# maxvonbuelow/harry

Hardware: AMD Instinct MI355X
Metric: Mtriangles/s encode+decode (higher is better)
Workload: dtype u8/u16 residual bytes, u32 range-coder registers (compat profile: u64)

## Files before the change

harry_amd/csrc/device/chunked.cpp:

```cpp
#include <chrono>
#include <condition_variable>
#include <cstdio>
#include <cstdlib>
#include <cstring>
#include <deque>
#include <memory>
#include <mutex>
#include <thread>

#include "codec_math.hpp"
#include "context.hpp"
#include "kernels.hpp"

namespace hry {

using namespace dev;
static const char kMarkPrefix[] = "[hry enc]";

static constexpr int kDefaultChunk = 8192;
static constexpr uint32_t kMaxChunk = 1u << 20;


static uint32_t stream_words(uint32_t n, uint32_t t0)
{
// ... 539 lines not shown
		std::vector<RestartCounters> scounters;
		dir.restarts = select_restart_points(w.marks, w.named, dir.counters, &w.snapshots, &scounters);
		if (!w.snapshots.empty()) write_snapshot_section(w.snapshot_faces, w.snapshots, scounters, dir.snapshot_section);
		write_restart_section(dir, restart_sec);
	};
	const bool dir_beside = w.marks.size() >= 4096 && host_threads() > 1;
	SideThreads dir_helper;
	if (dir_beside) dir_helper.spawn(select_restarts);

	const uint32_t vc = (uint32_t)w.order_v.size(), fc = (uint32_t)w.order_f.size();
	if (piped && (vc != pipe->vc || fc != pipe->fc)) throw Error(HRY_E_INTERNAL, "encode pipeline: sizes changed under the walk");
	if (chunk_syms <= 0) {
		uint64_t total = (uint64_t)w.n_conn + (uint64_t)vc * ldv.nplanes + (uint64_t)fc * ldf.nplanes;
		if (m.general) for (const AttrList &L : m.lists) total += (uint64_t)L.count * L.coded_bytes();
		while (CH < (1u << 15) && total / CH > 8192) CH <<= 1;
	}

	auto t_h2d = Clock::now();
	size_t op_plane_n[8];
	for (int k = 0; k < 8; ++k) op_plane_n[k] = w.n_op_class[k];
	size_t ngrp = 0, conn_plane_bytes = 0, nopb = w.op_sc.size();
	for (int g = 0; g < G_COUNT; ++g) { ngrp += w.grp_val[g].size(); conn_plane_bytes += w.grp_val[g].size() * kGroupBytes[g]; }
	cx.d_order_v.ensure(std::max<size_t>((size_t)vc * 4, 16));
	cx.d_order_f.ensure(std::max<size_t>((size_t)fc * 4, 16));
	cx.d_rank.ensure(std::max<size_t>((size_t)dev_nv * 4, 16));
	cx.d_grp_val.ensure(std::max<size_t>(ngrp * 4, 16));
	cx.d_connplanes.ensure(std::max<size_t>(conn_plane_bytes + 2 * nopb + 64, 16));
	cx.d_vplanes.ensure(std::max<size_t>((size_t)vc * ldv.nplanes, 16));
	cx.d_fplanes.ensure(std::max<size_t>((size_t)fc * ldf.nplanes, 16));
	const bool nt_piped = piped && pipe->nt != nullptr;
	if (vc && !piped) HIP_OK(hipMemcpyAsync(cx.d_order_v.p, w.order_v.data(), (size_t)vc * 4, hipMemcpyHostToDevice, cx.stream));
	if (fc && (ldf.nplanes || m.general) && !piped) HIP_OK(hipMemcpyAsync(cx.d_order_f.p, w.order_f.data(), (size_t)fc * 4, hipMemcpyHostToDevice, cx.stream));
	if (!piped) upload_repaired_twins(cx, in_place ? *in_place->whole : m, w, in_place != nullptr);
	if (in_place) cx.inplace_twin_patches.insert(cx.inplace_twin_patches.end(), w.twin_patches.begin(), w.twin_patches.end());
	size_t goff[G_COUNT + 1] = { 0 };
	for (int g = 0; g < G_COUNT; ++g) {
		size_t n = w.grp_val[g].size();
		goff[g + 1] = goff[g] + n;
		if (n && !(g == G_NUMTRI && nt_piped)) HIP_OK(hipMemcpyAsync(cx.d_grp_val.as<uint32_t>() + goff[g], w.grp_val[g].data(), n * 4, hipMemcpyHostToDevice, cx.stream));
	}
	uint8_t *d_opplanes = cx.d_connplanes.as<uint8_t>() + conn_plane_bytes;
	uint8_t *d_opraw = d_opplanes + nopb;
	if (nopb) HIP_OK(hipMemcpyAsync(d_opraw, w.op_sc.data(), nopb, hipMemcpyHostToDevice, cx.stream));

	const std::vector<GenPlane> layout = container_planes(m);
	std::vector<PlaneRef> planes;
	auto add_plane = [&](const uint8_t *at, uint32_t n) { planes.push_back(PlaneRef{ at, n, layout.at(planes.size()).init }); };
	{
		size_t poff = 0;
		for (int g = 0; g < G_COUNT; ++g) {
			uint32_t n = (uint32_t)w.grp_val[g].size();
			const uint8_t *at = g == G_NUMTRI && nt_piped ? cx.d_nt_planes.as<uint8_t>() : cx.d_connplanes.as<uint8_t>() + poff;
			for (int b = 0; b < kGroupBytes[g]; ++b) add_plane(at + (size_t)b * n, n);
			poff += (size_t)n * kGroupBytes[g];
		}
		size_t o = 0;
		for (int k = 0; k < kOpClasses; ++k) { add_plane(d_opplanes + o, (uint32_t)op_plane_n[k]); o += op_plane_n[k]; }
		for (int p = 0; p < ldv.nplanes; ++p) add_plane(cx.d_vplanes.as<uint8_t>() + (size_t)p * vc, vc);
		for (int p = 0; p < ldf.nplanes; ++p) add_plane(cx.d_fplanes.as<uint8_t>() + (size_t)p * fc, fc);
	}
	if (m.general) general_planes_encode(cx, m, w, planes);
	if (planes.size() != layout.size()) throw Error(HRY_E_INTERNAL, "chunked encode: the planes do not match the container's layout");
	std::vector<uint32_t> kind_tabs;
	build_init_tables(m, kind_tabs);
	const uint32_t CHC = std::min(CH, std::max(CH / 8, 512u));
	dir.CH = CH; dir.CHC = CHC;
	const uint32_t npl = (uint32_t)planes.size();
	std::vector<HistSlice> slices;
	for (uint32_t pi = 0; pi < npl; ++pi)
		for (uint32_t f = 0; f < planes[pi].n; f += 16384) slices.push_back(HistSlice{ planes[pi].dptr + f, std::min(16384u, planes[pi].n - f), pi });
	cx.d_small.ensure(std::max<size_t>(slices.size() * sizeof(HistSlice) + (size_t)npl * 1024 + 64, 64));
	uint32_t *d_hist = cx.d_small.as<uint32_t>();
	HistSlice *d_slices = (HistSlice*)(cx.d_small.as<uint8_t>() + (size_t)npl * 1024);
	if (!slices.empty()) HIP_OK(hipMemcpyAsync(d_slices, slices.data(), slices.size() * sizeof(HistSlice), hipMemcpyHostToDevice, cx.stream));
	HIP_OK(hipMemsetAsync(d_hist, 0, (size_t)npl * 1024, cx.stream));
	HIP_OK(hipStreamSynchronize(cx.stream));
	cx.timing.h2d_ms = ms_since(t_h2d);
	HRY_MARK(t_all, "walk's outputs on the device");

	ConnView cv = cx.conn_view();
	HIP_OK(hipEventRecord(cx.ev[1], cx.stream));
	if (!m.general && !piped) {
		HIP_OK(hipMemsetAsync(cx.d_rank.p, 0xff, (size_t)dev_nv * 4, cx.stream));
		launch_rank(cx.stream, cx.d_order_v.as<uint32_t>(), vc, cv.org, cx.d_rank.as<uint32_t>());
		launch_predict_vtx(cx.stream, cv, cx.d_order_v.as<uint32_t>(), vc, cx.d_rank.as<uint32_t>(), cx.d_rec[1].as<uint8_t>(), ldv, cx.d_vplanes.as<uint8_t>());
		launch_face_planes(cx.stream, cv, cx.d_order_f.as<uint32_t>(), fc, cx.d_rec[0].as<uint8_t>(), ldf, cx.d_fplanes.as<uint8_t>());
	}
	{
		size_t poff = 0;
		for (int g = 0; g < G_COUNT; ++g) {
			uint32_t n = (uint32_t)w.grp_val[g].size();
			if (!(g == G_NUMTRI && nt_piped)) launch_split_bytes(cx.stream, cx.d_grp_val.as<uint32_t>() + goff[g], n, kGroupBytes[g], cx.d_connplanes.as<uint8_t>() + poff);
			poff += (size_t)n * kGroupBytes[g];
		}
	}
	{
		uint32_t base[8], o = 0;
		for (int k = 0; k < 8; ++k) { base[k] = o; o += (uint32_t)op_plane_n[k]; }
		cx.d_op.ensure(((nopb + kSplitUnit - 1) / kSplitUnit + 1) * 8 * 4 + 64);
		launch_split_classes(cx.stream, d_opraw, (uint32_t)nopb, base, cx.d_op.as<uint32_t>(), d_opplanes);
	}
	launch_plane_hist(cx.stream, d_slices, (uint32_t)slices.size(), d_hist);
	HIP_OK(hipEventRecord(cx.ev[2], cx.stream));
	std::vector<uint32_t> hist((size_t)npl * 256);
	if (npl) HIP_OK(hipMemcpyAsync(hist.data(), d_hist, hist.size() * 4, hipMemcpyDeviceToHost, cx.stream));
	HIP_OK(hipStreamSynchronize(cx.stream));
	HRY_MARK(t_all, "planes and their histograms");

	dir.tables.assign((size_t)npl * 256, 0);
	dir.has_prior.assign(npl, 0);
	dir.nsym.resize(npl);
	std::vector<uint32_t> totals(npl, 0);
	for (uint32_t pi = 0; pi < npl; ++pi) {
		uint32_t *tab = dir.tables.data() + (size_t)pi * 256;
		const bool use = plane_prior_from_hist(hist.data() + (size_t)pi * 256, planes[pi].n, tab);
		if (!use) memcpy(tab, kind_tabs.data() + (size_t)planes[pi].init * 256, 1024);
		for (int i = 0; i < 256; ++i) totals[pi] += tab[i];
		dir.has_prior[pi] = use ? 1 : 0;
		dir.nsym[pi] = planes[pi].n;
	}
	std::vector<StreamJob> jobs;
	uint64_t words = 0;
	uint64_t nsym_total = 0;
	uint32_t max_t0 = 256;
	for (uint32_t pi = 0; pi < npl; ++pi) {
		const PlaneRef &pl = planes[pi];
		nsym_total += pl.n;
		max_t0 = std::max(max_t0, totals[pi]);
		for_plane_streams(pi, pl.n, CH, CHC, [&](uint64_t f, uint32_t n) {
			if (words >= (1ull << 32) - (1u << 24)) throw Error(HRY_E_UNSUPPORTED, "chunked stream accumulator exceeds 2^32 words");
			jobs.push_back(StreamJob{ pl.dptr + f, n, pi, totals[pi], (uint32_t)words });
			words += stream_words(n, totals[pi]);
		});
	}
	const uint32_t ns = (uint32_t)jobs.size();
	const uint32_t nw = (uint32_t)words + 2;
	HRY_MARK(t_all, "  priors and stream jobs (host)");
	cx.d_init.ensure(std::max<size_t>(dir.tables.size() * 4, 16));
	if (!dir.tables.empty()) HIP_OK(hipMemcpyAsync(cx.d_init.p, dir.tables.data(), dir.tables.size() * 4, hipMemcpyHostToDevice, cx.stream));
	cx.d_cjobs.ensure(std::max<size_t>((size_t)ns * sizeof(StreamJob), 16));
	if (ns) HIP_OK(hipMemcpyAsync(cx.d_cjobs.p, jobs.data(), (size_t)ns * sizeof(StreamJob), hipMemcpyHostToDevice, cx.stream));
	cx.ensure_magic(max_t0 + CH + 16);
	cx.d_acc.ensure((size_t)nw * 8);
	cx.d_summary.ensure(((size_t)nw / 1024 + 8) * 4);
	cx.d_bytes.ensure((size_t)nw * 4);
	cx.d_csizes.ensure(std::max<size_t>((size_t)ns * 8, 16));
	cx.d_coffs.ensure(((size_t)ns + 1) * 8);
	HIP_OK(hipMemsetAsync(cx.d_acc.p, 0, (size_t)nw * 8, cx.stream));
	uint32_t *d_bits = cx.d_csizes.as<uint32_t>(), *d_nbytes = d_bits + ns;
	bool split_kernels;
	{
		uint32_t longest = 0;
		for (uint32_t i = 0; i < ns; ++i) longest = std::max(longest, jobs[i].n);
		const double one = std::max(longest * 0.09e-3, (double)nsym_total * 0.04e-6), two = longest * 0.207e-3 + (double)nsym_total * 0.0057e-6;
		const uint64_t min_streams = env_uint("HRY_ENCODE_SPLIT_MIN_STREAMS", ~0ull);
		split_kernels = min_streams != ~0ull ? min_streams != 0 && ns >= min_streams : ns >= 64 && two < 0.9 * one;
	}
	for (uint32_t i = 0; i < ns && split_kernels; ++i) split_kernels = (uint64_t)jobs[i].t0 + jobs[i].n <= 65535u;
	std::vector<uint64_t> tab;
	if (split_kernels) {
		tab.resize((size_t)ns + ((size_t)ns + 1) / 2);
		uint32_t *order = (uint32_t*)(tab.data() + ns);
		uint64_t off = 0;
		for (uint32_t i = 0; i < ns; ++i) { tab[i] = off; off += jobs[i].n; order[i] = i; }
		std::stable_sort(order, order + ns, [&](uint32_t a, uint32_t b) { return jobs[a].n > jobs[b].n; });
		cx.d_rec_sym.ensure(std::max<size_t>((size_t)off * 8, 16));
		cx.d_split.ensure(tab.size() * 8);
		HIP_OK(hipMemcpyAsync(cx.d_split.p, tab.data(), tab.size() * 8, hipMemcpyHostToDevice, cx.stream));
		HIP_OK(hipEventRecord(cx.ev[3], cx.stream));
		launch_chunk_encode_split(cx.stream, cx.d_cjobs.as<StreamJob>(), ns, cx.d_init.as<uint32_t>(), cx.d_magic.as<MagicEnt>(), cx.d_acc.as<uint64_t>(), d_bits,
		                          cx.d_split.as<uint64_t>(), cx.d_rec_sym.p, (const uint32_t*)(cx.d_split.as<uint64_t>() + ns));
		HIP_OK(hipEventRecord(cx.ev[4], cx.stream));
	} else {
	HIP_OK(hipEventRecord(cx.ev[3], cx.stream));
	launch_chunk_encode(cx.stream, cx.d_cjobs.as<StreamJob>(), ns, cx.d_init.as<uint32_t>(), cx.d_magic.as<MagicEnt>(), cx.d_acc.as<uint64_t>(), d_bits);
	HIP_OK(hipEventRecord(cx.ev[4], cx.stream));
	}
	launch_carry(cx.stream, cx.d_acc.as<uint64_t>(), nw, cx.d_v.as<uint64_t>(), cx.d_summary.as<uint32_t>(), cx.d_bytes.as<uint8_t>(), cx.d_cjobs.as<StreamJob>(), d_bits, ns);
	launch_stream_pack(cx.stream, cx.d_cjobs.as<StreamJob>(), ns, d_bits, nullptr, d_nbytes, cx.d_coffs.as<uint64_t>(), nullptr, false);
	cx.h_small.ensure(64);
	volatile uint64_t *total_bytes_p = cx.h_small.as<uint64_t>();
	*total_bytes_p = 0;
	HIP_OK(hipMemcpyAsync((void*)total_bytes_p, cx.d_coffs.as<uint64_t>() + ns, 8, hipMemcpyDeviceToHost, cx.stream));
	HRY_MARK(t_all, "  stream kernels launched");
	if (dir_beside) dir_helper.rethrow(); else select_restarts();
	HRY_MARK(t_all, "  restart points selected");
	HIP_OK(hipStreamSynchronize(cx.stream));
	const uint64_t total_bytes = *total_bytes_p;
	HRY_MARK(t_all, "streams coded");
	cx.d_cout.ensure(std::max<size_t>(total_bytes, 16));
	launch_stream_pack(cx.stream, cx.d_cjobs.as<StreamJob>(), ns, d_bits, cx.d_bytes.as<uint8_t>(), d_nbytes, cx.d_coffs.as<uint64_t>(), cx.d_cout.as<uint8_t>(), true);
	HIP_OK(hipEventRecord(cx.ev[5], cx.stream));

	write_container(cx, dir, restart_sec, ns, d_nbytes, total_bytes, out);
	HRY_MARK(t_all, "container on the host");
	if (sharded) { const uint64_t seg_len = out.size() - seg_begin; memcpy(out.data() + seg_len_at, &seg_len, 8); }

	if (cx.keep_stages) {
		cx.stage_put_host("order_v", w.order_v.data(), (size_t)vc * 4);
		cx.stage_put_host("order_f", w.order_f.data(), (size_t)fc * 4);
		cx.stage_put("vplanes", cx.d_vplanes.p, (size_t)vc * ldv.nplanes);
		cx.stage_put("fplanes", cx.d_fplanes.p, (size_t)fc * ldf.nplanes);
		cx.stage_put("d_twin", cx.d_twin.p, (size_t)(in_place ? in_place->whole->ne() : m.ne()) * 4);
	}
	cx.timing.k_predict_ms = cx.elapsed(1, 2);
	cx.timing.k_entropy_ms = cx.elapsed(3, 4);
	cx.timing.device_ms = cx.elapsed(1, 5);
	cx.timing.n_symbols = nsym_total;
	cx.timing.payload_bytes = total_bytes;
	cx.timing.total_ms = ms_since(t_all);
}

Mesh *decode_chunked(Context &cx, const uint8_t *p, size_t n, size_t hdr, std::unique_ptr<Mesh> m);
Mesh *decode_compat(Context &cx, const uint8_t *p, size_t n, size_t hdr, std::unique_ptr<Mesh> m);

Mesh *decode_any(Context &cx, const uint8_t *p, size_t n, int shard_index, int shard_count, bool allow_partial)
{
	HIP_OK(hipSetDevice(cx.device));
	std::unique_ptr<Mesh> m(new Mesh());
	int minor = 0;
	const bool sharded = n >= 6 && p[4] == 0 && p[5] == 3;
	size_t hdr = read_hry_header(p, n, *m, minor, !sharded);
	if (minor == 3) { Context *one = &cx; return decode_sharded(&one, 1, p, n, hdr, std::move(m), shard_index, shard_count, allow_partial || shard_count > 1, nullptr); }
	if (shard_count > 1) throw Error(HRY_E_ARG, "only a sharded container (.hry v0.3) decodes segment by segment");
	if (minor == 2) return decode_chunked(cx, p, n, hdr, std::move(m));
	if (m->general) return decode_general(cx, p, n, hdr, std::move(m));
	return decode_compat(cx, p, n, hdr, std::move(m));
}

}
```

harry_amd/csrc/device/chunked.hip:

```cpp
#include <hip/hip_runtime.h>

#include <mutex>
#include <stdexcept>
#include <type_traits>

#include "codec_math.hpp"
#include "dev_types.hpp"
#include "kernels.hpp"

namespace hry {
namespace dev {

__device__ __forceinline__ uint32_t wscan_excl(uint32_t v, uint32_t &total)
{
	uint32_t inc = v;
#pragma unroll
	for (int d = 1; d < 64; d <<= 1) {
		uint32_t o = __shfl_up(inc, d, 64);
		if ((int)(threadIdx.x & 63) >= d) inc += o;
	}
	total = __shfl(inc, 63, 64);
	return inc - v;
}

constexpr int kWin = 72;

__global__ __launch_bounds__(64) void k_chunk_encode(const StreamJob *jobs, const uint32_t *inits, const MagicEnt *magic,
                                                     unsigned long long *acc, uint32_t *stream_bits)
{
	const StreamJob jb = jobs[blockIdx.x];
	const int lane = threadIdx.x;
	__shared__ uint32_t cnt[257], cum[257], bh[256];
	__shared__ unsigned long long win[kWin];
	{
		const uint32_t *st = inits + (size_t)jb.init * 256 + 4 * lane;
		uint32_t a = st[0], b = st[1], c = st[2], d = st[3], tot;
		uint32_t ex = wscan_excl(a + b + c + d, tot);
		cnt[4 * lane] = a; cnt[4 * lane + 1] = b; cnt[4 * lane + 2] = c; cnt[4 * lane + 3] = d;
		cum[4 * lane] = ex; cum[4 * lane + 1] = ex + a; cum[4 * lane + 2] = ex + a + b; cum[4 * lane + 3] = ex + a + b + c;
		if (lane == 0) { cnt[256] = 0; cum[256] = 0; }
	}
	__syncthreads();
	uint32_t R = 1u << 31;
	uint32_t S = 0;
	const uint64_t earlier = lane == 0 ? 0ull : (~0ull >> (64 - lane));
	for (uint32_t base = 0; base < jb.n; base += 64) {
		const uint32_t j = base + lane;
		const bool valid = j < jb.n;
		const uint32_t nb = min(64u, jb.n - base);
		const uint32_t s = valid ? jb.sym[j] : 0x100u;
		uint64_t eq = ~0ull, lt = 0;
#pragma unroll
		for (int b = 8; b >= 0; --b) {
			const bool mine = (s >> b) & 1u;
			const uint64_t m = __ballot(mine);
			lt |= mine ? (eq & ~m) : 0ull;
			eq &= mine ? m : ~m;
		}
		const uint32_t l = cum[s] + (uint32_t)__popcll(lt & earlier), c = cnt[s] + (uint32_t)__popcll(eq & earlier);
		const uint32_t t = jb.t0 + j;
		const bool sub = l + c == t;
		MagicEnt me = valid ? magic[t] : MagicEnt{ 0, 0, 0 };
		const uint32_t mx = valid ? (sub ? l : c) : 0u;
		const uint32_t mm = ((me.shift >> kMagicSh32Shift) & 31u) | (sub || !valid ? 0x80u : 0u);
		uint32_t my_r = 0, my_s = 0;
		const uint32_t s_first = S;
		auto step = [&](uint32_t i) {
			const uint32_t M = (uint32_t)__builtin_amdgcn_readlane((int)me.m32, (int)i);
			const uint32_t x = (uint32_t)__builtin_amdgcn_readlane((int)mx, (int)i);
			const uint32_t meta = (uint32_t)__builtin_amdgcn_readlane((int)mm, (int)i);
			const uint32_t r = __umulhi(R, M) >> (meta & 31u);
			const uint32_t prod = r * x;
			const uint32_t Rn = (meta & 0x80u) ? R - prod : prod;
			const uint32_t y = Rn - 1u;
			const uint32_t sh = y ? (uint32_t)__builtin_clz(y) - 1u : 31u;
			my_r = lane == (int)i ? r : my_r;
			my_s = lane == (int)i ? S : my_s;
			R = Rn << sh;
			S += sh;
		};
		uint32_t i = 0;
		for (; i + 4 <= nb; i += 4) { step(i); step(i + 1); step(i + 2); step(i + 3); }
		for (; i < nb; ++i) step(i);
		const uint32_t w0 = s_first >> 5, span = ((S + 63) >> 5) - w0 + 1;
		const uint32_t a = (valid && l) ? my_r * l : 0u;
		const uint32_t w = my_s >> 5, shb = my_s & 31;
		const uint32_t hi = a >> shb, lo = shb ? a << (32 - shb) : 0u;
		unsigned long long *dst = acc + jb.word_base;
		for (uint32_t k = lane; k < span; k += 64) win[k] = 0;
		bh[4 * lane] = 0; bh[4 * lane + 1] = 0; bh[4 * lane + 2] = 0; bh[4 * lane + 3] = 0;
		__syncthreads();
		if (hi) atomicAdd(&win[w - w0], (unsigned long long)hi);
		if (lo) atomicAdd(&win[w - w0 + 1], (unsigned long long)lo);
		if (valid) atomicAdd(&bh[s], 1u);
		__syncthreads();
		for (uint32_t k = lane; k < span; k += 64) {
			unsigned long long v = win[k];
			if (v) atomicAdd(&dst[w0 + k], v);
		}
		uint32_t a0 = bh[4 * lane], a1 = bh[4 * lane + 1], a2 = bh[4 * lane + 2], a3 = bh[4 * lane + 3], tot;
		uint32_t ex = wscan_excl(a0 + a1 + a2 + a3, tot);
		cnt[4 * lane] += a0; cnt[4 * lane + 1] += a1; cnt[4 * lane + 2] += a2; cnt[4 * lane + 3] += a3;
		cum[4 * lane] += ex; cum[4 * lane + 1] += ex + a0; cum[4 * lane + 2] += ex + a0 + a1; cum[4 * lane + 3] += ex + a0 + a1 + a2;
		__syncthreads();
	}
	if (lane == 0) stream_bits[blockIdx.x] = S + 32;
}

__global__ __launch_bounds__(64) void k_chunk_model(const StreamJob *jobs, const uint32_t *inits, const MagicEnt *magic, const unsigned long long *rec_off, uint2 *rec)
{
	const StreamJob jb = jobs[blockIdx.x];
	const int lane = threadIdx.x;
	__shared__ uint32_t cnt[257], cum[257], bh[256];
	{
		const uint32_t *st = inits + (size_t)jb.init * 256 + 4 * lane;
		uint32_t a = st[0], b = st[1], c = st[2], d = st[3], tot;
		uint32_t ex = wscan_excl(a + b + c + d, tot);
		cnt[4 * lane] = a; cnt[4 * lane + 1] = b; cnt[4 * lane + 2] = c; cnt[4 * lane + 3] = d;
		cum[4 * lane] = ex; cum[4 * lane + 1] = ex + a; cum[4 * lane + 2] = ex + a + b; cum[4 * lane + 3] = ex + a + b + c;
		if (lane == 0) { cnt[256] = 0; cum[256] = 0; }
	}
	__syncthreads();
	uint2 *out = rec + rec_off[blockIdx.x];
	const uint64_t earlier = lane == 0 ? 0ull : (~0ull >> (64 - lane));
	for (uint32_t base = 0; base < jb.n; base += 64) {
		const uint32_t j = base + lane;
		const bool valid = j < jb.n;
		const uint32_t s = valid ? jb.sym[j] : 0x100u;
		uint64_t eq = ~0ull, lt = 0;
#pragma unroll
		for (int b = 8; b >= 0; --b) {
			const bool mine = (s >> b) & 1u;
			const uint64_t m = __ballot(mine);
			lt |= mine ? (eq & ~m) : 0ull;
			eq &= mine ? m : ~m;
		}
		const uint32_t l = cum[s] + (uint32_t)__popcll(lt & earlier), c = cnt[s] + (uint32_t)__popcll(eq & earlier);
		if (valid) {
			const MagicEnt me = magic[jb.t0 + j];
			const uint32_t msh = (me.shift >> kMagicSh32Shift) & 31u;
			const uint32_t q = me.m32 == 0x80000000u ? me.m32 >> msh : (me.m32 - 1u) >> msh;
			out[j] = make_uint2(l | (c << 16), q);
		}
		bh[4 * lane] = 0; bh[4 * lane + 1] = 0; bh[4 * lane + 2] = 0; bh[4 * lane + 3] = 0;
		__syncthreads();
		if (valid) atomicAdd(&bh[s], 1u);
		__syncthreads();
		uint32_t a0 = bh[4 * lane], a1 = bh[4 * lane + 1], a2 = bh[4 * lane + 2], a3 = bh[4 * lane + 3], tot;
		uint32_t ex = wscan_excl(a0 + a1 + a2 + a3, tot);
		cnt[4 * lane] += a0; cnt[4 * lane + 1] += a1; cnt[4 * lane + 2] += a2; cnt[4 * lane + 3] += a3;
		cum[4 * lane] += ex; cum[4 * lane + 1] += ex + a0; cum[4 * lane + 2] += ex + a0 + a1; cum[4 * lane + 3] += ex + a0 + a1 + a2;
		__syncthreads();
	}
}

__global__ __launch_bounds__(64) void k_chunk_ranges(const StreamJob *jobs, uint32_t njobs, const uint32_t *order, const unsigned long long *rec_off,
                                                     const uint2 *rec, unsigned long long *acc, uint32_t *stream_bits)
{
	__shared__ uint32_t tile_lc[64 * 65], tile_q[64 * 65];
	const uint32_t lane = threadIdx.x;
	const uint32_t slot = blockIdx.x * 64 + lane;
	const bool have = slot < njobs;
	const uint32_t job = have ? order[slot] : 0u;
	StreamJob jb{ nullptr, 0, 0, 256, 0 };
	if (have) jb = jobs[job];
	const uint32_t n = have ? jb.n : 0u;
	const uint2 *in = rec + (have ? rec_off[job] : 0ull);
	unsigned long long *dst = acc + jb.word_base;
	uint32_t nmax = n;
#pragma unroll
	for (int d = 32; d >= 1; d >>= 1) nmax = max(nmax, (uint32_t)__shfl_xor((int)nmax, d, 64));
	nmax = (uint32_t)__builtin_amdgcn_readfirstlane((int)nmax);
	const uint32_t in_lo = (uint32_t)(uintptr_t)in, in_hi = (uint32_t)((uintptr_t)in >> 32);
	uint2 nxt[64];
	auto fetch = [&](uint32_t step0) {
#pragma unroll
		for (int s = 0; s < 64; ++s) {
			const uint32_t ns = (uint32_t)__builtin_amdgcn_readlane((int)n, s);
			const uint2 *ps = (const uint2*)(((uintptr_t)(uint32_t)__builtin_amdgcn_readlane((int)in_hi, s) << 32) | (uint32_t)__builtin_amdgcn_readlane((int)in_lo, s));
			const uint32_t j = step0 + lane;
			nxt[s] = j < ns ? ps[j] : make_uint2(0u, 0u);
		}
	};
	auto stash = [&]() {
#pragma unroll
		for (int s = 0; s < 64; ++s) { tile_lc[s * 65 + lane] = nxt[s].x; tile_q[s * 65 + lane] = nxt[s].y; }
	};
	uint32_t R = 1u << 31, S = 0, t = jb.t0;
	uint32_t cur_w = 0;
	unsigned long long a0 = 0, a1 = 0;
	fetch(0);
	stash();
	for (uint32_t step0 = 0; step0 < nmax; step0 += 64) {
		const bool more = step0 + 64 < nmax;
		if (more) fetch(step0 + 64);
		const uint32_t *row_lc = tile_lc + lane * 65, *row_q = tile_q + lane * 65;
		const uint32_t left = nmax - step0 < 64u ? nmax - step0 : 64u;
		for (uint32_t k = 0; k < left; ++k) {
			const uint32_t lc = row_lc[k], q = row_q[k];
			const bool live = step0 + k < n;
			const uint32_t l = lc & 0xffffu, c = lc >> 16;
			uint32_t r = __umulhi(R, q);
			r += R - r * t >= t ? 1u : 0u;
			uint32_t rl, rc;
			asm("v_mul_lo_u32 %0, %1, %2" : "=v"(rl) : "v"(r), "v"(l));
			asm("v_mul_lo_u32 %0, %1, %2" : "=v"(rc) : "v"(r), "v"(c));
			const uint32_t Rn = l + c == t ? R - rl : rc;
			const uint32_t w = S >> 5;
			const unsigned long long two = ((unsigned long long)(live ? rl : 0u) << 32) >> (S & 31u);
			if (w != cur_w) { dst[cur_w] = a0; a0 = a1; a1 = 0; cur_w = w; }
			a0 += two >> 32;
			a1 += two & 0xffffffffull;
			const uint32_t y = Rn - 1u;
			const uint32_t sh = y ? (uint32_t)__builtin_clz(y) - 1u : 31u;
			R = live ? Rn << sh : R;
			S += live ? sh : 0u;
			t += live ? 1u : 0u;
		}
		if (more) stash();
	}
	if (have) {
		dst[cur_w] = a0;
		dst[cur_w + 1u] = a1;
		stream_bits[job] = S + 32u;
	}
}

__global__ __launch_bounds__(1024) void k_stream_offsets(const uint32_t *stream_bits, uint32_t n, uint32_t *nbytes, unsigned long long *offsets)
{
	__shared__ unsigned long long wave_tot[16];
	__shared__ unsigned long long carry;
	if (threadIdx.x == 0) carry = 0;
	__syncthreads();
	const int lane = threadIdx.x & 63, wv = threadIdx.x >> 6;
	for (uint32_t base = 0; base < n; base += 1024) {
		uint32_t i = base + threadIdx.x;
		uint32_t nb = i < n ? (stream_bits[i] + 7) >> 3 : 0;
		unsigned long long inc = nb;
#pragma unroll
		for (int d = 1; d < 64; d <<= 1) {
			unsigned long long o = __shfl_up(inc, d, 64);
			if (lane >= d) inc += o;
		}
		if (lane == 63) wave_tot[wv] = inc;
		__syncthreads();
		unsigned long long pre = carry;
		for (int k = 0; k < wv; ++k) pre += wave_tot[k];
		if (i < n) { nbytes[i] = nb; offsets[i] = pre + inc - nb; }
		__syncthreads();
		if (threadIdx.x == 1023) carry = pre + inc;
		__syncthreads();
	}
	if (threadIdx.x == 0) offsets[n] = carry;
}

__global__ __launch_bounds__(256) void k_pack_streams(const StreamJob *jobs, const uint8_t *bytes, const uint32_t *nbytes, const unsigned long long *offsets, uint8_t *out)
{
	const StreamJob jb = jobs[blockIdx.x];
// ... 131 lines not shown
	for (int d = 32; d >= 1; d >>= 1) nmax = max(nmax, (uint32_t)__shfl_xor((int)nmax, d, 64));
	nmax = (uint32_t)__builtin_amdgcn_readfirstlane((int)nmax);
	MagicEnt me = magic[t];
	uint32_t o0 = 0, o1 = 0, o2 = 0, o3 = 0;
	for (uint32_t i = 0; i < nmax; ++i) {
		if ((i & 15u) == 0u && i) {
			if (i < jb.n) {
				typedef uint32_t u32x4 __attribute__((ext_vector_type(4)));
				typedef __attribute__((address_space(1))) u32x4 __attribute__((aligned(1))) gvec;
				*(gvec*)(out + i - 16) = u32x4{ o0, o1, o2, o3 };
			}
		}
		if (i >= jb.n) continue;
		const uint32_t r = __umulhi(R, me.m32) >> ((me.shift >> kMagicSh32Shift) & 31u);
		me = magic[t + 1u];
		uint32_t q = (uint32_t)((float)D * __builtin_amdgcn_rcpf((float)r));
		int32_t rem = (int32_t)(D - __umul24(q, r));
		if (rem < 0) { --q; rem += (int32_t)r; }
		if (rem < 0) { --q; rem += (int32_t)r; }
		if (rem >= (int32_t)r) { ++q; rem -= (int32_t)r; }
		if (rem >= (int32_t)r) { ++q; rem -= (int32_t)r; }
		const uint32_t target = min(t - 1u, q);
		uint32_t b = 0, lo = 0;
#pragma unroll
		for (int k = 0; k < 16; ++k) {
			const bool le = C[k] <= target;
			b += le ? 1u : 0u;
			lo = le ? C[k] : lo;
		}
		const CT *cb = cnt + (size_t)(b * 16u) * 64 + lane;
		uint32_t sin = 0, run = lo, hi = 0xffffffffu;
#pragma unroll
		for (int k = 0; k < 16; ++k) {
			run += (uint32_t)cb[k * 64];
			const bool le = run <= target;
			sin += le ? 1u : 0u;
			lo = le ? run : lo;
			hi = min(hi, le ? 0xffffffffu : run);
		}
		const uint32_t s = b * 16u + sin;
		const uint32_t cs = hi - lo;
		const uint32_t rl = __umul24(r, lo);
		const uint32_t Rn = hi < t ? __umul24(r, cs) : R - rl;
		const uint32_t y = Rn - 1u;
		const uint32_t sh = y ? (uint32_t)__builtin_clz(y) - 1u : 31u;
		R = Rn << sh;
		if (avail < 32u) { buf |= (uint64_t)ahead << (32u - avail); avail += 32u; ahead = word_at(p); p += 4u; }
		const uint32_t bits = (uint32_t)((buf >> 1) >> (63u - sh));
		buf <<= sh; avail -= sh;
		D = ((D - rl) << sh) | bits;
		cnt[s * 64 + lane] = (CT)(cs + 1u);
#pragma unroll
		for (int k = 0; k < 16; ++k) C[k] += (uint32_t)k >= b ? 1u : 0u;
		++t;
		o0 = __builtin_amdgcn_alignbyte(o1, o0, 1); o1 = __builtin_amdgcn_alignbyte(o2, o1, 1); o2 = __builtin_amdgcn_alignbyte(o3, o2, 1);
		o3 = (o3 >> 8) | (s << 24);
		if (i + 1u == jb.n) {
			const uint32_t m = jb.n & 15u ? jb.n & 15u : 16u;
			auto shift = [&] { o0 = __builtin_amdgcn_alignbyte(o1, o0, 1); o1 = __builtin_amdgcn_alignbyte(o2, o1, 1); o2 = __builtin_amdgcn_alignbyte(o3, o2, 1); o3 >>= 8; };
			for (uint32_t k = m; k < 16u; ++k) shift();
			for (uint32_t k = 0; k < m; ++k) { out[jb.n - m + k] = (uint8_t)o0; shift(); }
		}
	}
}

__global__ __launch_bounds__(256) void k_scatter_u32(const uint32_t *pairs, uint32_t n, uint32_t *dst)
{
	uint32_t i = blockIdx.x * blockDim.x + threadIdx.x;
	if (i < n) dst[pairs[2 * i]] = pairs[2 * i + 1];
}

__global__ __launch_bounds__(256) void k_plane_hist(const HistSlice *slices, uint32_t *hist)
{
	const HistSlice sl = slices[blockIdx.x];
	__shared__ uint32_t bins[256];
	bins[threadIdx.x] = 0;
	__syncthreads();
	for (uint32_t i = threadIdx.x; i < sl.n; i += 256) atomicAdd(&bins[sl.sym[i]], 1u);
	__syncthreads();
	if (bins[threadIdx.x]) atomicAdd(&hist[(size_t)sl.plane * 256 + threadIdx.x], bins[threadIdx.x]);
}

__global__ __launch_bounds__(64) void k_split_count(const uint8_t *ops, uint32_t n, uint32_t *cnt)
{
	const uint32_t u = blockIdx.x, lane = threadIdx.x;
	uint32_t c[8] = { 0, 0, 0, 0, 0, 0, 0, 0 };
	for (uint32_t i = u * kSplitUnit + lane; i < min(n, (u + 1) * kSplitUnit); i += 64) {
		const uint32_t k = ops[i] >> 3;
#pragma unroll
		for (int j = 0; j < 8; ++j) c[j] += k == (uint32_t)j;
	}
#pragma unroll
	for (int j = 0; j < 8; ++j) {
		uint32_t v = c[j];
		for (int m = 32; m > 0; m >>= 1) v += __shfl_xor(v, m);
		if (lane == 0) cnt[u * 8 + j] = v;
	}
}
__global__ __launch_bounds__(64) void k_split_scan(uint32_t *cnt, uint32_t nunits, SplitBase base)
{
	const uint32_t j = blockIdx.x, lane = threadIdx.x;
	uint32_t run = base.b[j];
	for (uint32_t u0 = 0; u0 < nunits; u0 += 64) {
		const uint32_t u = u0 + lane;
		const uint32_t c = u < nunits ? cnt[u * 8 + j] : 0u;
		uint32_t inc = c;
		for (int d = 1; d < 64; d <<= 1) { const uint32_t o = __shfl_up(inc, d); if ((int)lane >= d) inc += o; }
		if (u < nunits) cnt[u * 8 + j] = run + inc - c;
		run += __shfl(inc, 63);
	}
}
__global__ __launch_bounds__(64) void k_split_place(const uint8_t *ops, uint32_t n, const uint32_t *cnt, uint8_t *planes)
{
	const uint32_t u = blockIdx.x, lane = threadIdx.x;
	uint32_t at[8];
#pragma unroll
	for (int j = 0; j < 8; ++j) at[j] = cnt[u * 8 + j];
	const uint32_t end = min(n, (u + 1) * kSplitUnit);
	for (uint32_t i0 = u * kSplitUnit; i0 < end; i0 += 64) {
		const uint32_t i = i0 + lane;
		const bool live = i < end;
		const uint32_t b = live ? ops[i] : 0xffu, k = b >> 3;
		uint32_t dst = 0;
#pragma unroll
		for (int j = 0; j < 8; ++j) {
			const uint64_t mk = __ballot(live && k == (uint32_t)j);
			if (live && k == (uint32_t)j) dst = at[j] + (uint32_t)__popcll(mk & ((1ull << lane) - 1ull));
			at[j] += (uint32_t)__popcll(mk);
		}
		if (live) planes[dst] = (uint8_t)(b & 7u);
	}
}
void launch_split_classes(hipStream_t st, const uint8_t *ops, uint32_t n, const uint32_t base[8], uint32_t *scratch, uint8_t *planes)
{
	if (!n) return;
	const uint32_t nunits = (n + kSplitUnit - 1) / kSplitUnit;
	SplitBase sb;
	for (int j = 0; j < 8; ++j) sb.b[j] = base[j];
	hipLaunchKernelGGL(k_split_count, dim3(nunits), dim3(64), 0, st, ops, n, scratch);
	hipLaunchKernelGGL(k_split_scan, dim3(8), dim3(64), 0, st, scratch, nunits, sb);
	hipLaunchKernelGGL(k_split_place, dim3(nunits), dim3(64), 0, st, ops, n, scratch, planes);
}

void launch_plane_hist(hipStream_t st, const HistSlice *slices, uint32_t nslices, uint32_t *hist)
{
	if (nslices) hipLaunchKernelGGL(k_plane_hist, dim3(nslices), dim3(256), 0, st, slices, hist);
}
void launch_scatter_u32(hipStream_t st, const uint32_t *pairs, uint32_t n, uint32_t *dst)
{
	if (n) hipLaunchKernelGGL(k_scatter_u32, dim3((n + 255) / 256), dim3(256), 0, st, pairs, n, dst);
}
void launch_chunk_encode(hipStream_t st, const StreamJob *jobs, uint32_t nstreams, const uint32_t *inits, const MagicEnt *magic, uint64_t *acc, uint32_t *stream_bits)
{
	if (nstreams) hipLaunchKernelGGL(k_chunk_encode, dim3(nstreams), dim3(64), 0, st, jobs, inits, magic, (unsigned long long*)acc, stream_bits);
}
void launch_chunk_encode_split(hipStream_t st, const StreamJob *jobs, uint32_t nstreams, const uint32_t *inits, const MagicEnt *magic, uint64_t *acc, uint32_t *stream_bits,
                               const uint64_t *rec_off, void *rec, const uint32_t *order)
{
	if (!nstreams) return;
	hipLaunchKernelGGL(k_chunk_model, dim3(nstreams), dim3(64), 0, st, jobs, inits, magic, (const unsigned long long*)rec_off, (uint2*)rec);
	hipLaunchKernelGGL(k_chunk_ranges, dim3((nstreams + 63) / 64), dim3(64), 0, st, jobs, nstreams, order, (const unsigned long long*)rec_off, (const uint2*)rec,
	                   (unsigned long long*)acc, stream_bits);
}
void launch_stream_pack(hipStream_t st, const StreamJob *jobs, uint32_t nstreams, const uint32_t *stream_bits, const uint8_t *bytes,
                        uint32_t *nbytes, uint64_t *offsets, uint8_t *out, bool pack)
{
	if (!pack) hipLaunchKernelGGL(k_stream_offsets, dim3(1), dim3(1024), 0, st, stream_bits, nstreams, nbytes, (unsigned long long*)offsets);
	else if (nstreams) hipLaunchKernelGGL(k_pack_streams, dim3(nstreams), dim3(256), 0, st, jobs, bytes, nbytes, (const unsigned long long*)offsets, out);
}
void launch_scatter_u8(hipStream_t st, const uint8_t *src, const uint32_t *dst_index, uint32_t n, uint8_t *dst)
{
	if (n) hipLaunchKernelGGL(k_scatter_u8, dim3((n + 255) / 256), dim3(256), 0, st, src, dst_index, n, dst);
}
void launch_chunk_decode(hipStream_t st, const StreamJob *jobs, uint32_t nstreams, const uint32_t *inits, const MagicEnt *magic,
                         const uint8_t *payload, const uint64_t *offsets, const uint32_t *nbytes)
{
	if (nstreams) hipLaunchKernelGGL(k_chunk_decode, dim3(nstreams), dim3(64), 0, st, jobs, inits, magic, payload, (const unsigned long long*)offsets, nbytes, (uint8_t*)nullptr);
}
template <typename CT>
static void launch_chunk_decode_lanes_as(hipStream_t st, const StreamJob *jobs, uint32_t nstreams, const uint32_t *inits, const MagicEnt *magic,
                                         const uint8_t *payload, const uint64_t *offsets, const uint32_t *nbytes)
{
	constexpr uint32_t kLds = 256 * 64 * sizeof(CT);
	static std::mutex mu;
	static bool raised[64] = {};
	int dev = 0;
	if (hipGetDevice(&dev) != hipSuccess || dev < 0 || dev >= 64) dev = 0;
	{
		std::lock_guard<std::mutex> g(mu);
		if (!raised[dev]) {
			if (hipFuncSetAttribute((const void*)k_chunk_decode_lanes<CT>, hipFuncAttributeMaxDynamicSharedMemorySize, (int)kLds) != hipSuccess) {
				(void)hipGetLastError();
				throw std::runtime_error("k_chunk_decode_lanes: the device refuses its dynamic LDS");
			}
			raised[dev] = true;
		}
	}
	hipLaunchKernelGGL(k_chunk_decode_lanes<CT>, dim3((nstreams + 63) / 64), dim3(64), kLds, st, jobs, nstreams, inits, magic, payload, (const unsigned long long*)offsets, nbytes);
	if (hipGetLastError() != hipSuccess) throw std::runtime_error("k_chunk_decode_lanes: launch failed");
}
void launch_chunk_decode_lanes(hipStream_t st, const StreamJob *jobs, uint32_t nstreams, const uint32_t *inits, const MagicEnt *magic,
                               const uint8_t *payload, const uint64_t *offsets, const uint32_t *nbytes, bool counts16)
{
	if (!nstreams) return;
	if (counts16) launch_chunk_decode_lanes_as<uint16_t>(st, jobs, nstreams, inits, magic, payload, offsets, nbytes);
	else launch_chunk_decode_lanes_as<uint32_t>(st, jobs, nstreams, inits, magic, payload, offsets, nbytes);
}

}
}
```

Before: 59.85.

## Split chunk encoder into model and range-coder wavefronts with double-buffered handoff

```diff
diff --git a/harry_amd/csrc/device/chunked.cpp b/harry_amd/csrc/device/chunked.cpp
--- a/harry_amd/csrc/device/chunked.cpp
+++ b/harry_amd/csrc/device/chunked.cpp
@@ -715,7 +715,7 @@
 	{
 		uint32_t longest = 0;
 		for (uint32_t i = 0; i < ns; ++i) longest = std::max(longest, jobs[i].n);
-		const double one = std::max(longest * 0.09e-3, (double)nsym_total * 0.04e-6), two = longest * 0.207e-3 + (double)nsym_total * 0.0057e-6;
+		const double one = std::max(longest * 0.045e-3, (double)nsym_total * 0.03e-6), two = longest * 0.207e-3 + (double)nsym_total * 0.0057e-6;
 		const uint64_t min_streams = env_uint("HRY_ENCODE_SPLIT_MIN_STREAMS", ~0ull);
 		split_kernels = min_streams != ~0ull ? min_streams != 0 && ns >= min_streams : ns >= 64 && two < 0.9 * one;
 	}
diff --git a/harry_amd/csrc/device/chunked.hip b/harry_amd/csrc/device/chunked.hip
--- a/harry_amd/csrc/device/chunked.hip
+++ b/harry_amd/csrc/device/chunked.hip
@@ -3,6 +3,7 @@
 #include <mutex>
 #include <stdexcept>
 #include <type_traits>
+#include <utility>
 
 #include "codec_math.hpp"
 #include "dev_types.hpp"
@@ -23,87 +24,167 @@
 	return inc - v;
 }
 
+__device__ __forceinline__ uint32_t wscan_excl_dpp(uint32_t v)
+{
+	int inc = (int)v;
+	inc += __builtin_amdgcn_update_dpp(0, inc, 0x111, 0xf, 0xf, false);
+	inc += __builtin_amdgcn_update_dpp(0, inc, 0x112, 0xf, 0xf, false);
+	inc += __builtin_amdgcn_update_dpp(0, inc, 0x114, 0xf, 0xf, false);
+	inc += __builtin_amdgcn_update_dpp(0, inc, 0x118, 0xf, 0xf, false);
+	inc += __builtin_amdgcn_update_dpp(0, inc, 0x142, 0xa, 0xf, false);
+	inc += __builtin_amdgcn_update_dpp(0, inc, 0x143, 0xc, 0xf, false);
+	return (uint32_t)inc - v;
+}
+
+template <uint32_t... I, typename F>
+__device__ __forceinline__ void for_each_lane(std::integer_sequence<uint32_t, I...>, F &f) { (f(std::integral_constant<uint32_t, I>()), ...); }
+
 constexpr int kWin = 72;
 
-__global__ __launch_bounds__(64) void k_chunk_encode(const StreamJob *jobs, const uint32_t *inits, const MagicEnt *magic,
-                                                     unsigned long long *acc, uint32_t *stream_bits)
+#ifdef HRY_ENCODE_CLOCKS
+#define HRY_ECLK(...) __VA_ARGS__
+#else
+#define HRY_ECLK(...)
+#endif
+
+__device__ __forceinline__ void wave_sync()
+{
+	__builtin_amdgcn_fence(__ATOMIC_RELEASE, "workgroup");
+	__builtin_amdgcn_wave_barrier();
+	__builtin_amdgcn_fence(__ATOMIC_ACQUIRE, "workgroup");
+}
+
+__global__ __launch_bounds__(128) void k_chunk_encode(const StreamJob *jobs, const uint32_t *inits, const MagicEnt *magic,
+                                                      unsigned long long *acc, uint32_t *stream_bits)
 {
 	const StreamJob jb = jobs[blockIdx.x];
-	const int lane = threadIdx.x;
+	const int lane = threadIdx.x & 63;
+	const bool model_wave = __builtin_amdgcn_readfirstlane((int)(threadIdx.x >> 6)) == 0;
 	__shared__ uint32_t cnt[257], cum[257], bh[256];
 	__shared__ unsigned long long win[kWin];
-	{
-		const uint32_t *st = inits + (size_t)jb.init * 256 + 4 * lane;
-		uint32_t a = st[0], b = st[1], c = st[2], d = st[3], tot;
-		uint32_t ex = wscan_excl(a + b + c + d, tot);
-		cnt[4 * lane] = a; cnt[4 * lane + 1] = b; cnt[4 * lane + 2] = c; cnt[4 * lane + 3] = d;
-		cum[4 * lane] = ex; cum[4 * lane + 1] = ex + a; cum[4 * lane + 2] = ex + a + b; cum[4 * lane + 3] = ex + a + b + c;
-		if (lane == 0) { cnt[256] = 0; cum[256] = 0; }
-	}
-	__syncthreads();
+	__shared__ uint32_t q_m32[2][64], q_x[2][64], q_meta[2][64], q_l[2][64];
+	if (model_wave) {
+		{
+			const uint32_t *st = inits + (size_t)jb.init * 256 + 4 * lane;
+			uint32_t a = st[0], b = st[1], c = st[2], d = st[3], tot;
+			uint32_t ex = wscan_excl(a + b + c + d, tot);
+			cnt[4 * lane] = a; cnt[4 * lane + 1] = b; cnt[4 * lane + 2] = c; cnt[4 * lane + 3] = d;
+			cum[4 * lane] = ex; cum[4 * lane + 1] = ex + a; cum[4 * lane + 2] = ex + a + b; cum[4 * lane + 3] = ex + a + b + c;
+			if (lane == 0) { cnt[256] = 0; cum[256] = 0; }
+		}
+		wave_sync();
+		const uint64_t earlier = lane == 0 ? 0ull : (~0ull >> (64 - lane));
+		typedef __attribute__((address_space(1))) const uint8_t gsym;
+		gsym *const sym = (gsym*)jb.sym;
+		uint32_t s_next = (uint32_t)lane < jb.n ? (uint32_t)sym[lane] : 0x100u;
+		MagicEnt me_next = (uint32_t)lane < jb.n ? magic[jb.t0 + lane] : MagicEnt{ 0, 0, 0 };
+		asm volatile("" : : "v"(s_next), "v"(me_next.shift), "v"(me_next.m32));
+		HRY_ECLK(unsigned long long ck_model = 0, ck_update = 0, ck_loads = 0, ck_wait = 0, ck_n = 0;)
+		for (uint32_t base = 0, par = 0; base < jb.n; base += 64, par ^= 1u) {
+			HRY_ECLK(const unsigned long long ck0 = __builtin_amdgcn_s_memtime();)
+			const uint32_t j = base + lane;
+			const bool valid = j < jb.n;
+			const uint32_t s = s_next;
+			const MagicEnt me = me_next;
+			{
+				const uint32_t jn = j + 64;
+				const bool more = jn < jb.n;
+				s_next = more ? (uint32_t)sym[jn] : 0x100u;
+				me_next = more ? magic[jb.t0 + jn] : MagicEnt{ 0, 0, 0 };
+			}
+			uint64_t eq = ~0ull, lt = 0;
+#pragma unroll
+			for (int b = 8; b >= 0; --b) {
+				const bool mine = (s >> b) & 1u;
+				const uint64_t m = __ballot(mine);
+				lt |= mine ? (eq & ~m) : 0ull;
+				eq &= mine ? m : ~m;
+			}
+			const uint32_t l = cum[s] + (uint32_t)__popcll(lt & earlier), c = cnt[s] + (uint32_t)__popcll(eq & earlier);
+			const uint32_t t = jb.t0 + j;
+			const bool sub = l + c == t;
+			q_m32[par][lane] = me.m32;
+			q_x[par][lane] = valid ? (sub ? l : c) : 0u;
+			q_meta[par][lane] = ((me.shift >> kMagicSh32Shift) & 31u) | (sub || !valid ? 0x80000000u : 0u);
+			q_l[par][lane] = valid ? l : 0u;
+			HRY_ECLK(wave_sync(); const unsigned long long ck1 = __builtin_amdgcn_s_memtime();)
+			bh[4 * lane] = 0; bh[4 * lane + 1] = 0; bh[4 * lane + 2] = 0; bh[4 * lane + 3] = 0;
+			wave_sync();
+			if (valid) atomicAdd(&bh[s], 1u);
+			wave_sync();
+			uint32_t a0 = bh[4 * lane], a1 = bh[4 * lane + 1], a2 = bh[4 * lane + 2], a3 = bh[4 * lane + 3];
+			uint32_t ex = wscan_excl_dpp(a0 + a1 + a2 + a3);
+			cnt[4 * lane] += a0; cnt[4 * lane + 1] += a1; cnt[4 * lane + 2] += a2; cnt[4 * lane + 3] += a3;
+			cum[4 * lane] += ex; cum[4 * lane + 1] += ex + a0; cum[4 * lane + 2] += ex + a0 + a1; cum[4 * lane + 3] += ex + a0 + a1 + a2;
+			HRY_ECLK(wave_sync(); const unsigned long long ck2 = __builtin_amdgcn_s_memtime();)
+			asm volatile("" : : "v"(s_next), "v"(me_next.shift), "v"(me_next.m32));
+			HRY_ECLK(const unsigned long long ck3 = __builtin_amdgcn_s_memtime();)
+			__syncthreads();
+			HRY_ECLK({ const unsigned long long ck4 = __builtin_amdgcn_s_memtime(); ck_model += ck1 - ck0; ck_update += ck2 - ck1; ck_loads += ck3 - ck2; ck_wait += ck4 - ck3; ++ck_n; })
+		}
+		HRY_ECLK(if (lane == 0 && jb.n >= 4096 && (blockIdx.x & 31) == 0)
+		             printf("k_chunk_encode stream %u, %u symbols, model wavefront, ticks a batch: model %llu, table update %llu, wait for the next loads %llu, wait at the barrier %llu\n",
+		                    blockIdx.x, jb.n, ck_model / ck_n, ck_update / ck_n, ck_loads / ck_n, ck_wait / ck_n);)
+		return;
+	}
 	uint32_t R = 1u << 31;
 	uint32_t S = 0;
-	const uint64_t earlier = lane == 0 ? 0ull : (~0ull >> (64 - lane));
-	for (uint32_t base = 0; base < jb.n; base += 64) {
-		const uint32_t j = base + lane;
-		const bool valid = j < jb.n;
+	unsigned long long *dst = acc + jb.word_base;
+	HRY_ECLK(unsigned long long ck_wait = 0, ck_steps = 0, ck_flush = 0, ck_n = 0;)
+	for (uint32_t base = 0, par = 0; base < jb.n; base += 64, par ^= 1u) {
 		const uint32_t nb = min(64u, jb.n - base);
-		const uint32_t s = valid ? jb.sym[j] : 0x100u;
-		uint64_t eq = ~0ull, lt = 0;
-#pragma unroll
-		for (int b = 8; b >= 0; --b) {
-			const bool mine = (s >> b) & 1u;
-			const uint64_t m = __ballot(mine);
-			lt |= mine ? (eq & ~m) : 0ull;
-			eq &= mine ? m : ~m;
-		}
-		const uint32_t l = cum[s] + (uint32_t)__popcll(lt & earlier), c = cnt[s] + (uint32_t)__popcll(eq & earlier);
-		const uint32_t t = jb.t0 + j;
-		const bool sub = l + c == t;
-		MagicEnt me = valid ? magic[t] : MagicEnt{ 0, 0, 0 };
-		const uint32_t mx = valid ? (sub ? l : c) : 0u;
-		const uint32_t mm = ((me.shift >> kMagicSh32Shift) & 31u) | (sub || !valid ? 0x80u : 0u);
-		uint32_t my_r = 0, my_s = 0;
+		HRY_ECLK(const unsigned long long ck0 = __builtin_amdgcn_s_memtime();)
+		__syncthreads();
+		HRY_ECLK(const unsigned long long ck1 = __builtin_amdgcn_s_memtime();)
+		const uint32_t m32 = q_m32[par][lane], mx = q_x[par][lane], mm = q_meta[par][lane], l = q_l[par][lane];
+		uint32_t my_R = 0;
 		const uint32_t s_first = S;
-		auto step = [&](uint32_t i) {
-			const uint32_t M = (uint32_t)__builtin_amdgcn_readlane((int)me.m32, (int)i);
+		auto step = [&](auto lane_i) {
+			const uint32_t i = lane_i;
+			const uint32_t M = (uint32_t)__builtin_amdgcn_readlane((int)m32, (int)i);
 			const uint32_t x = (uint32_t)__builtin_amdgcn_readlane((int)mx, (int)i);
-			const uint32_t meta = (uint32_t)__builtin_amdgcn_readlane((int)mm, (int)i);
-			const uint32_t r = __umulhi(R, M) >> (meta & 31u);
+			const int32_t meta = __builtin_amdgcn_readlane((int)mm, (int)i);
+			const uint32_t r = __umulhi(R, M) >> ((uint32_t)meta & 31u);
 			const uint32_t prod = r * x;
-			const uint32_t Rn = (meta & 0x80u) ? R - prod : prod;
-			const uint32_t y = Rn - 1u;
-			const uint32_t sh = y ? (uint32_t)__builtin_clz(y) - 1u : 31u;
-			my_r = lane == (int)i ? r : my_r;
-			my_s = lane == (int)i ? S : my_s;
-			R = Rn << sh;
-			S += sh;
+			const uint32_t Rn = meta < 0 ? R - prod : prod;
+			uint32_t y;
+			asm("s_lshl1_add_u32 %0, %1, -1" : "=s"(y) : "s"(Rn) : "scc");
+			if constexpr (std::is_same<decltype(lane_i), uint32_t>::value)
+				my_R = lane == (int)i ? R : my_R;
+			else
+				asm("v_writelane_b32 %0, %1, %2" : "+v"(my_R) : "s"(R), "n"(decltype(lane_i)::value));
+			R = Rn << (uint32_t)__builtin_clz(y);
 		};
-		uint32_t i = 0;
-		for (; i + 4 <= nb; i += 4) { step(i); step(i + 1); step(i + 2); step(i + 3); }
-		for (; i < nb; ++i) step(i);
+		if (nb == 64u) {
+			for_each_lane(std::make_integer_sequence<uint32_t, 64>(), step);
+		} else {
+			for (uint32_t i = 0; i < nb; ++i) step(i);
+		}
+		HRY_ECLK(asm volatile("" : : "s"(R), "v"(my_R)); const unsigned long long ck2 = __builtin_amdgcn_s_memtime();)
+		const uint32_t my_r = __umulhi(my_R, m32) >> (mm & 31u);
+		const uint32_t my_Rn = (int32_t)mm < 0 ? my_R - my_r * mx : my_r * mx;
+		const uint32_t my_sh = (uint32_t)__builtin_clz(2u * my_Rn - 1u);
+		const uint32_t my_s = s_first + wscan_excl_dpp(my_sh);
+		S = (uint32_t)__builtin_amdgcn_readlane((int)(my_s + my_sh), 63);
 		const uint32_t w0 = s_first >> 5, span = ((S + 63) >> 5) - w0 + 1;
-		const uint32_t a = (valid && l) ? my_r * l : 0u;
+		const uint32_t a = l ? my_r * l : 0u;
 		const uint32_t w = my_s >> 5, shb = my_s & 31;
 		const uint32_t hi = a >> shb, lo = shb ? a << (32 - shb) : 0u;
-		unsigned long long *dst = acc + jb.word_base;
 		for (uint32_t k = lane; k < span; k += 64) win[k] = 0;
-		bh[4 * lane] = 0; bh[4 * lane + 1] = 0; bh[4 * lane + 2] = 0; bh[4 * lane + 3] = 0;
-		__syncthreads();
+		wave_sync();
 		if (hi) atomicAdd(&win[w - w0], (unsigned long long)hi);
 		if (lo) atomicAdd(&win[w - w0 + 1], (unsigned long long)lo);
-		if (valid) atomicAdd(&bh[s], 1u);
-		__syncthreads();
+		wave_sync();
 		for (uint32_t k = lane; k < span; k += 64) {
 			unsigned long long v = win[k];
 			if (v) atomicAdd(&dst[w0 + k], v);
 		}
-		uint32_t a0 = bh[4 * lane], a1 = bh[4 * lane + 1], a2 = bh[4 * lane + 2], a3 = bh[4 * lane + 3], tot;
-		uint32_t ex = wscan_excl(a0 + a1 + a2 + a3, tot);
-		cnt[4 * lane] += a0; cnt[4 * lane + 1] += a1; cnt[4 * lane + 2] += a2; cnt[4 * lane + 3] += a3;
-		cum[4 * lane] += ex; cum[4 * lane + 1] += ex + a0; cum[4 * lane + 2] += ex + a0 + a1; cum[4 * lane + 3] += ex + a0 + a1 + a2;
-		__syncthreads();
-	}
+		wave_sync();
+		HRY_ECLK({ const unsigned long long ck3 = __builtin_amdgcn_s_memtime(); ck_wait += ck1 - ck0; ck_steps += ck2 - ck1; ck_flush += ck3 - ck2; ++ck_n; })
+	}
+	HRY_ECLK(if (lane == 0 && jb.n >= 4096 && (blockIdx.x & 31) == 0)
+	             printf("k_chunk_encode stream %u, %u symbols, range wavefront, ticks a batch: wait at the barrier %llu, records and 64 steps %llu, window to the accumulators %llu\n",
+	                    blockIdx.x, jb.n, ck_wait / ck_n, ck_steps / ck_n, ck_flush / ck_n);)
 	if (lane == 0) stream_bits[blockIdx.x] = S + 32;
 }
 
@@ -541,7 +622,7 @@
 }
 void launch_chunk_encode(hipStream_t st, const StreamJob *jobs, uint32_t nstreams, const uint32_t *inits, const MagicEnt *magic, uint64_t *acc, uint32_t *stream_bits)
 {
-	if (nstreams) hipLaunchKernelGGL(k_chunk_encode, dim3(nstreams), dim3(64), 0, st, jobs, inits, magic, (unsigned long long*)acc, stream_bits);
+	if (nstreams) hipLaunchKernelGGL(k_chunk_encode, dim3(nstreams), dim3(128), 0, st, jobs, inits, magic, (unsigned long long*)acc, stream_bits);
 }
 void launch_chunk_encode_split(hipStream_t st, const StreamJob *jobs, uint32_t nstreams, const uint32_t *inits, const MagicEnt *magic, uint64_t *acc, uint32_t *stream_bits,
                                const uint64_t *rec_off, void *rec, const uint32_t *order)
```

New measurement: 59.75, median of 2. About the same (-0.2%).
